# ChuWeiEr/GravInv3DHMC

Measured on AMD Instinct MI355X. Metric: HMC leapfrog steps/sec + G·ρ achieved HBM GB/s at 1/2/4/8 GPUs, higher is better.
Workload: dtype f64

## Files before the change

gravinv3dhmc_amd/_lib.py:

```python
import ctypes as C
import os

import numpy as np

_HERE = os.path.dirname(os.path.abspath(__file__))
LIB_PATH = os.environ.get("GRAVHMC_LIB") or os.path.join(_HERE, "libgravhmc.so")

GH_OK, GH_ERR_ARG, GH_ERR_HIP, GH_ERR_NOMEM, GH_ERR_OVERFLOW, GH_ERR_UNSUPPORTED, GH_ERR_COMM = \
    0, -1, -2, -3, -4, -5, -6
CELL_PRISM, CELL_TESSEROID, CELL_PRISM_TF, CELL_PRISM_COMP, CELL_TESSEROID_COMP, CELL_PRISM_JOINT = 0, 1, 2, 3, 4, 5
CELL_PRISM_MULTI = 6
CELL_PRISM_MVI = 7
CELL_PRISM_MVI_DATA = 8
CELL_TESS_MVI_DATA = 9
CELL_TESSEROID_MULTI = 10
BCOMP_TF, BCOMP_BX, BCOMP_BY, BCOMP_BZ = range(4)
BCOMPONENTS = {"tf": BCOMP_TF, "bx": BCOMP_BX, "by": BCOMP_BY, "bz": BCOMP_BZ}
BCOMP_MAX = 4
MULTI_MAX = 11
COMP_POTENTIAL, COMP_GEOID, COMP_GX, COMP_GY, COMP_GZ, COMP_GXX, COMP_GXY, COMP_GXZ, COMP_GYY, COMP_GYZ, COMP_GZZ = \
    range(11)
COMPONENTS = {"potential": COMP_POTENTIAL, "geoid": COMP_GEOID, "gx": COMP_GX, "gy": COMP_GY, "gz": COMP_GZ,
              "gxx": COMP_GXX, "gxy": COMP_GXY, "gxz": COMP_GXZ, "gyy": COMP_GYY, "gyz": COMP_GYZ, "gzz": COMP_GZZ}
REG_KINDS = {"Damping": 0, "Smoothness": 1, "MS": 2, "TV": 3}
# ... 111 lines not shown
    "gh_shard_unique_id": (C.c_int, [C.c_void_p]),
    "gh_shard_init": (C.c_int, [_ctx, C.c_void_p, C.c_int, C.c_int, _i64, _i64]),
    "gh_shard_init_callback": (C.c_int, [_ctx, C.c_void_p, C.c_void_p, C.c_int, C.c_int, _i64, _i64]),
    "gh_shard_init_rows": (C.c_int, [_ctx, C.c_void_p, C.c_int, C.c_int, _i64, _i64]),
    "gh_shard_init_rows_callback": (C.c_int, [_ctx, C.c_void_p, C.c_void_p, C.c_int, C.c_int, _i64, _i64]),
    "gh_shard_allreduce": (C.c_int, [_ctx, _dp, _i64]),
    "gh_rng_create": (C.c_int, [C.POINTER(C.c_void_p), C.c_uint32]),
    "gh_rng_destroy": (None, [C.c_void_p]),
    "gh_rng_set_threads": (C.c_int, [C.c_void_p, C.c_int]),
    "gh_host_cores": (C.c_int, []),
    "gh_rng_set_state": (C.c_int, [C.c_void_p, C.POINTER(C.c_uint32), C.c_int, C.c_int, C.c_double]),
    "gh_rng_get_state": (C.c_int, [C.c_void_p, C.POINTER(C.c_uint32), C.POINTER(C.c_int), C.POINTER(C.c_int),
                                   C.POINTER(C.c_double)]),
    "gh_rng_draw_trajectories": (C.c_int, [C.c_void_p, C.c_int, C.c_int, C.c_int, _i64, C.c_double,
                                           C.POINTER(C.c_int), _dp, _dp]),
    "gh_format_row_fixed8": (C.c_int64, [_dp, _i64, C.c_char_p, _i64]),
    "gh_measure_stream_read": (C.c_int, [_ctx, C.c_int, C.c_int, C.POINTER(C.c_double)]),
    "gh_profile_enable": (C.c_int, [_ctx, C.c_int]),
    "gh_fold_info": (C.c_int, [_ctx, C.POINTER(C.c_int), C.POINTER(C.c_int), C.POINTER(_i64), C.POINTER(C.c_double),
                               C.POINTER(C.c_double)]),
    "gh_fold_detect": (C.c_int, [_i64, _dp, _dp, _dp, _i64, _dp, C.POINTER(C.c_int), C.POINTER(C.c_int)]),
    "gh_fold_pair_info": (C.c_int, [_ctx, C.POINTER(C.c_int), C.POINTER(C.c_int), C.POINTER(_i64), C.POINTER(_i64),
                                    C.POINTER(_i64)]),
    "gh_fold_detect_pair": (C.c_int, [_i64, _dp, _dp, _dp, _i64, _dp, C.POINTER(C.c_int), C.POINTER(C.c_int),
                                      C.POINTER(C.c_int), C.POINTER(_i64), C.POINTER(C.c_int)]),
    "gh_fold_pair_rows": (C.c_int, [_i64, _dp, _dp, _dp, _i64, _dp, C.POINTER(C.c_int), C.POINTER(C.c_int),
                                    C.POINTER(C.c_int), C.POINTER(C.c_int), C.POINTER(_i64), C.POINTER(C.c_int)]),
    "gh_profile_read": (C.c_int, [_ctx, C.POINTER(C.c_double), C.POINTER(_i64),
                                  C.POINTER(_i64)]),
    "gh_set_translation_invariant": (C.c_int, [_ctx, C.c_int]),
# ... 62 lines not shown
```

gravinv3dhmc_amd/csrc/gravhmc.hip:

```cpp
#include "../../include/gravhmc.h"
#include "kernels.hip.h"
#include "batch.hip.h"
#include "bscg.hip.h"
#include "exchange.hip.h"
#include "resident.hip.h"
#include "resbatch.hip.h"
#include "teamsweep.hip.h"
#include "mfbatch.hip.h"
#include "batchteam.hip.h"
#include "lonsym.hip.h"
#include "lonsymh.hip.h"
#include "lonres.hip.h"
#include "lonsymw.hip.h"
#include "fold.hip.h"
#include "lattice.hip.h"
#include "latbatch.hip.h"
#include "poststream.hip.h"
#include "tessmag.hip.h"

#include <dlfcn.h>
#include <rccl/rccl.h>

#include <algorithm>
#include <array>
#include <atomic>
#include <cfloat>
#include <chrono>
#include <climits>
#include <cmath>
#include <cstdarg>
#include <cstdio>
#include <cstdlib>
#include <cstring>
#include <functional>
#include <map>
#include <mutex>
#include <string>
#include <utility>
#include <thread>
#include <vector>

using namespace ghk;
static_assert(COMP_POTENTIAL == GH_COMP_POTENTIAL && COMP_GEOID == GH_COMP_GEOID && COMP_GX == GH_COMP_GX &&
                  COMP_GY == GH_COMP_GY && COMP_GZ == GH_COMP_GZ && COMP_GXX == GH_COMP_GXX && COMP_GXY == GH_COMP_GXY &&
                  COMP_GXZ == GH_COMP_GXZ && COMP_GYY == GH_COMP_GYY && COMP_GYZ == GH_COMP_GYZ &&
                  COMP_GZZ == GH_COMP_GZZ,
              "the kernels' component numbers are the C ABI's GH_COMP_*");
static_assert(MULTI_MAX == GH_MULTI_MAX, "the kernels' row-block table holds the C ABI's GH_MULTI_MAX components");
static_assert(BCOMP_MAX == GH_BCOMP_MAX && BCOMP_MAX <= MULTI_MAX && BCOMP_TF == GH_BCOMP_TF && BCOMP_BX == GH_BCOMP_BX &&
                  BCOMP_BY == GH_BCOMP_BY && BCOMP_BZ == GH_BCOMP_BZ,
              "the kernels' data components are the C ABI's GH_BCOMP_*");

#include "host_rows.h"
#include "host_ctx.h"
#include "host_cells.h"
#include "host_sweep.h"
#include "host_fold.h"
#include "host_lattice.h"
#include "host_lonsym.h"
#include "host_comm.h"
#include "host_wavelet.h"
#include "host_eval.h"
#include "host_poststream.h"
#include "host_resident.h"
#include "host_resbatch.h"
#include "host_lonres.h"
#include "host_batch.h"
#include "host_batchrun.h"
// ... 49 lines not shown
    if (c->stream) hipStreamSynchronize(c->stream);
    if (c->sh.comm) {
        std::string err;
        RcclApi *api = rccl_api(err);
        if (api && api->CommDestroy) api->CommDestroy(c->sh.comm);
    }
    if (c->sh.hbuf) hipHostFree(c->sh.hbuf);
    if (c->bt.h) hipHostFree(c->bt.h);
    traj_lists_free(c->rs.lists);
    traj_lists_free(c->rs.ls.lists);
    if (c->ls) {
        traj_lists_free(c->ls->res.lists);
        if (c->ls->res.ev0) hipEventDestroy(c->ls->res.ev0);
        if (c->ls->res.ev1) hipEventDestroy(c->ls->res.ev1);
    }
    for (PinnedBlock &pm : c->pinned) hipHostFree(pm.base);
    for (void *p : c->allocs) hipFree(p);
    if (c->h_scal) hipHostFree(c->h_scal);
    for (hipEvent_t ev : c->ev) hipEventDestroy(ev);
    if (c->copy_ev) hipEventDestroy(c->copy_ev);
    if (c->copy_stream) hipStreamDestroy(c->copy_stream);
    if (c->rs.ev0) hipEventDestroy(c->rs.ev0);
    if (c->rs.ev1) hipEventDestroy(c->rs.ev1);
    if (c->stream) hipStreamDestroy(c->stream);
    delete c->ls;
    delete c->lat;
    delete c;
}

int gh_device_info(const gh_ctx *c, char *name256, int *cus, int64_t *mem_bytes)
// ... 1426 lines not shown
    HIPCHK(c, hipMemsetAsync(c->wv.coeff, 0, sizeof(double) * (size_t)c->wv.Mp, c->stream));
    TRY(run_dwt(c, c->tmpM, c->M, 1, c->wv.coeff, c->wv.s1, c->wv.s2));
    return d2h(c, coeff, c->wv.coeff, (size_t)c->wv.Mp);
}

int gh_forward_wavelet(gh_ctx *c, const double *mw, double *dpre)
{
    if (!c || !mw || !dpre) return fail(c, GH_ERR_ARG, "gh_forward_wavelet: null pointer");
    TRY(need(c, c->wv.on, "gh_forward_wavelet: call gh_compress_wavelet first"));
    HIPCHK(c, hipSetDevice(c->device));
    TRY(h2d(c, c->tmpM, mw, (size_t)c->M));
    TRY(wavelet_forward(c, c->tmpM, c->tmpN));
    return d2h(c, dpre, c->tmpN, (size_t)c->N);
}

int gh_chain_init(gh_ctx *c, const double *x0, const double *low, const double *high)
{
    if (!c || !x0 || !low || !high) return fail(c, GH_ERR_ARG, "gh_chain_init: null pointer");
    TRY(need(c, c->have_G && c->have_data && c->have_reg,
             "gh_chain_init: needs a kernel matrix, gh_set_data and gh_set_reg"));
    HIPCHK(c, hipSetDevice(c->device));
    TRY(ensure_work(c));
    c->cur = 0;
    c->xcur = 0;
    c->spec_valid = c->pn_valid = false;
    c->st_stale = false;
    c->accept_count = 0;
    TRY(h2d(c, c->xb[0], x0, (size_t)c->M));
    TRY(h2d(c, c->low, low, (size_t)c->M));
    TRY(h2d(c, c->high, high, (size_t)c->M));
    TRY(eval_forward(c, c->xb[0], c->st[0]));
    TRY(scal_ready(c, c->st[0]));
    TRY(d2h(c, c->h_scal, c->st[0].scal, 4));
    c->cg.phi_cur = 0.0;
    if (coupling_on(c)) {
        TRY(d2h(c, c->h_scal + 8, c->st[0].phi, 1));
        c->cg.phi_cur = c->h_scal[8];
    }
    c->cg.phi_last = c->cg.phi_cur;
    TRY(lonsym_epilogue_check(c));
    c->U_cur[0] = c->h_scal[2];
    c->U_cur[1] = c->h_scal[0];
    c->U_cur[2] = c->h_scal[1];
    c->chain_ready = true;
    return GH_OK;
}

int gh_chain_prefetch_momentum(gh_ctx *c, const double *p0_next)
{
    if (!c || !p0_next) return fail(c, GH_ERR_ARG, "gh_chain_prefetch_momentum: null pointer");
    TRY(need(c, c->chain_ready, "gh_chain_prefetch_momentum: call gh_chain_init first"));
    HIPCHK(c, hipSetDevice(c->device));
    TRY(h2d(c, c->pn, p0_next, (size_t)c->M));
    sumsq_kernel<<<dim3(c->n_pp0), dim3(256), 0, c->stream>>>(c->pn, c->M, c->pp0_part);
    {
        std::vector<double> part((size_t)c->n_pp0);
        TRY(d2h(c, part.data(), c->pp0_part, (size_t)c->n_pp0));
        double s = 0.0;
        for (double v : part) s += v;
// ... 489 lines not shown
    const gh_ctx::Resident::LockStep &b = c->rs.ls;
    if (launches) *launches = b.launches;
    if (lock_steps) *lock_steps = b.lock_steps;
    if (chain_steps) *chain_steps = b.chain_steps;
    if (lost_steps) *lost_steps = b.lost;
    if (timeouts) *timeouts = b.xg.aborts;
    return GH_OK;
}

int gh_pinned_alloc(gh_ctx *c, size_t bytes, void **host)
{
    if (!c || !host || bytes == 0) return fail(c, GH_ERR_ARG, "gh_pinned_alloc: null pointer or no bytes");
    HIPCHK(c, hipSetDevice(c->device));
    void *p = nullptr;
    HIPCHK(c, hipHostMalloc(&p, bytes));
    c->pinned.push_back({(char *)p, bytes});
    *host = p;
    return GH_OK;
}

int gh_pinned_free(gh_ctx *c, void *host)
{
    if (!c || !host) return fail(c, GH_ERR_ARG, "gh_pinned_free: null pointer");
    for (size_t i = 0; i < c->pinned.size(); ++i)
        if (c->pinned[i].base == (char *)host) {
            HIPCHK(c, hipSetDevice(c->device));
            if (c->stream) HIPCHK(c, hipStreamSynchronize(c->stream));
            HIPCHK(c, hipHostFree(host));
            c->pinned.erase(c->pinned.begin() + (long)i);
            return GH_OK;
// ... 301 lines not shown
    std::vector<std::thread> th;
    for (int t = 1; t < T; ++t) th.emplace_back(work, t);
    work(0);
    for (std::thread &x : th) x.join();
    int64_t pos = 0;
    for (int t = 0; t < T; ++t) {
        if (len[(size_t)t] < 0 || pos + len[(size_t)t] > cap) return -1;
        memcpy(out + pos, buf[(size_t)t].data(), (size_t)len[(size_t)t]);
        pos += len[(size_t)t];
    }
    return pos;
}

#include "host_rng.h"

int gh_profile_enable(gh_ctx *c, int enable)
{
    if (!c) return GH_ERR_ARG;
    HIPCHK(c, hipSetDevice(c->device));
    if (enable && c->ev.empty()) {
        c->ev.resize(8192);
        for (auto &e : c->ev) HIPCHK(c, hipEventCreate(&e));
        c->ev_bytes.assign(c->ev.size() / 2, 0);
    }
    for (gh_ctx *k : c->kids) TRY(gh_profile_enable(k, enable));
    c->prof = enable != 0;
    c->prof_stride = (c->ld * c->M * 8 < (int64_t)(1 << 30)) ? 16 : 1;
    c->prof_seen = 0;
    c->ev_used = 0;
    c->prof_ms_acc = 0.0;
// ... 147 lines not shown
```

gravinv3dhmc_amd/csrc/host_chain.h:

```cpp
#pragma once

static int chain_state_fresh(gh_ctx *c)
{
    if (!c->st_stale) return GH_OK;
    TRY(eval_forward(c, c->xb[c->xcur], c->st[c->cur]));
    TRY(scal_ready(c, c->st[c->cur]));
    TRY(d2h(c, c->h_scal, c->st[c->cur].scal, 4));
    c->U_cur[0] = c->h_scal[2];
    c->U_cur[1] = c->h_scal[0];
    c->U_cur[2] = c->h_scal[1];
    c->st_stale = false;
    return GH_OK;
}

static inline int other_of3(int a, int b)
{
    for (int i = 0; i < 3; ++i)
        if (i != a && i != b) return i;
    return 0;
}

static int chain_trajectory_impl(gh_ctx *c, const double *p0, double dt, int L, double u, const double *p0_next,
                                 int *accepted, double out5[5])
{
    if (!c || !p0 || !accepted || !out5) return fail(c, GH_ERR_ARG, "gh_chain_trajectory: null pointer");
    TRY(need(c, c->chain_ready, "gh_chain_trajectory: call gh_chain_init first"));
    if (L < 1) return fail(c, GH_ERR_ARG, "gh_chain_trajectory: L must be >= 1");
    HIPCHK(c, hipSetDevice(c->device));
    TRY(chain_state_fresh(c));
    struct TeamsOk {
        gh_ctx *c;
        ~TeamsOk() { c->chain_teams_ok = false; }
    } teams_guard{c};
    c->chain_teams_ok = true;
    const size_t M = (size_t)c->M;
    const int nt = c->n_teams;
    const bool use_spec = c->spec_valid && c->spec_dt == dt && p0[0] == c->spec_probe[0] &&
// ... 29 lines not shown
        a.low = c->low;
        a.high = c->high;
        a.c_u = (s == 0) ? dt * 0.5 : dt;
        a.dt = dt;
        a.slab = c->slab;
        TRY(launch_sweep(c, a));
        TRY(finalize(c, c->xb[xout], c->st[sout]));
        xin = xout;
        pin ^= 1;
        sin = sout;
    }
    bool spec = c->pn_valid;
    double probe[3] = {c->pn_probe[0], c->pn_probe[1], c->pn_probe[2]};
    double pn_pp0 = c->pn_pp0;
    bool pn_deferred = false;
    if (p0_next) {
        if (!c->copy_stream) {
            HIPCHK(c, hipStreamCreateWithFlags(&c->copy_stream, hipStreamNonBlocking));
            HIPCHK(c, hipEventCreateWithFlags(&c->copy_ev, hipEventDisableTiming));
        }
        HIPCHK(c, hipMemcpyAsync(c->pn, p0_next, M * sizeof(double), hipMemcpyHostToDevice, c->copy_stream));
        HIPCHK(c, hipEventRecord(c->copy_ev, c->copy_stream));
        HIPCHK(c, hipStreamWaitEvent(c->stream, c->copy_ev, 0));
        sumsq_kernel<<<dim3(c->n_pp0), dim3(256), 0, c->stream>>>(c->pn, c->M, c->pn0_part);
        probe[0] = p0_next[0];
        probe[1] = p0_next[c->M / 2];
        probe[2] = p0_next[c->M - 1];
        spec = true;
        pn_deferred = true;
    }
// ... 34 lines not shown
                                 c->stream));
    }
    if (!use_spec)
        HIPCHK(c, hipMemcpyAsync(h + 16 + 2 * nt, c->pp0_part, (size_t)c->n_pp0 * sizeof(double),
                                 hipMemcpyDeviceToHost, c->stream));
    if (pn_deferred)
        HIPCHK(c, hipMemcpyAsync(h + 16 + 2 * nt + c->n_pp0, c->pn0_part, (size_t)c->n_pp0 * sizeof(double),
                                 hipMemcpyDeviceToHost, c->stream));
    HIPCHK(c, hipStreamSynchronize(c->stream));
    TRY(lonsym_epilogue_check(c));
    bool failed = false;
    TRY(team_failed(c, &failed));
    if (!failed) TRY(mft_failed(c, &failed));
    auto redo = [&]() -> int {
        c->spec_valid = c->pn_valid = false;
        const int rc = chain_trajectory_impl(c, p0, dt, L, u, p0_next, accepted, out5);
        team_resume(c);
        return rc;
    };
    if (failed && c->sh.kind == 0) return redo();
    if (pn_deferred) {
        double s = 0.0;
        for (int t = 0; t < c->n_pp0; ++t) s += h[16 + 2 * nt + c->n_pp0 + t];
        pn_pp0 = s;
    }
    double pp1 = 0.0, pp0 = 0.0;
    for (int t = 0; t < nt; ++t) pp1 += h[16 + t];
    if (use_spec)
        pp0 = c->spec_pp0;
    else
        for (int t = 0; t < c->n_pp0; ++t) pp0 += h[16 + 2 * nt + t];
// ... 22 lines not shown
            c->spec_x = xs;
            c->spec_p = pin ^ 1;
            c->spec_set = ss;
            c->spec_probe[0] = probe[0];
            c->spec_probe[1] = probe[1];
            c->spec_probe[2] = probe[2];
        }
    } else if (spec) {
        c->spec_misses += 1;
    }
    c->pn_valid = false;
    *accepted = acc ? 1 : 0;
    c->cg.phi_last = c->cg.phi_cur;
    return GH_OK;
}
```

gravinv3dhmc_amd/csrc/host_ctx.h:

```cpp
#pragma once

static thread_local std::string g_create_error;

struct LonSymHost;
struct LatticeHost;

struct DevBuf {
    void *p = nullptr;
    size_t bytes = 0;
};

struct ExchangeGuard {
    unsigned *abort_w = nullptr;
    unsigned seen[4] = {0, 0, 0, 0};
    unsigned tag = 0, tagE = 0, ltag = 0;
    std::vector<DevBuf> grans;
    bool dirty = false;
    bool inflight = false;
    int aborts = 0;
};

struct TrajLists {
    int cap = 0;
    int *L = nullptr, *accepted = nullptr, *chain = nullptr;
// ... 309 lines not shown
        size_t lds = 0;
        double max_dev = 0.0, build_ms = 0.0;
        int64_t launches = 0;
        bool exact = false;
        bool pair_detected = false, pair_on = false;
        int pair_reason = GH_FOLD_PAIR_UNDECIDED;
        int64_t n_work = 0, n_pairs = 0, work_per_team = 0;
        int pair_rows = 0;
        bool pair_rows_ok = false;
        int *wtab_d = nullptr, *row_tau_d = nullptr, *orb_tau_d = nullptr;
        int *ptab_d = nullptr, *row_code_d = nullptr;
    } fd;

    std::vector<PinnedBlock> pinned;

    double *ring = nullptr, *ring_mean = nullptr, *ring_sd = nullptr;
    int ring_K = 0, ring_next = 0;
    int64_t ring_count = 0;

    struct PostStream {
        bool on = false;
        int slot = 0;
        int64_t from = 0, count = 0;
        ghk::PostState d = {};
        double *lo = nullptr, *hi = nullptr, *iw = nullptr;
        double *row = nullptr;
        double *out = nullptr;
        double *qout = nullptr;
        size_t qout_n = 0;
        int64_t n[16] = {}, K[16] = {};
// ... 192 lines not shown
```

gravinv3dhmc_amd/csrc/host_rng.h:

```cpp
#pragma once

static const int RNG_BLOCKS = 8;

#if defined(__x86_64__) && !defined(__HIP_DEVICE_COMPILE__)
#define GH_HOST_CLONES __attribute__((target_clones("avx512f", "avx2", "default")))
#else
#define GH_HOST_CLONES
#endif

struct gh_rng {
    uint32_t keys[RNG_BLOCKS][624];
    uint32_t out[RNG_BLOCKS * 624];
    int nb;
    int p;
    int has_gauss;
    double gauss;
    std::vector<double> r2;
    int threads = 0;
};

GH_HOST_CLONES static void rng_twist(const uint32_t *in, uint32_t *mt)
{
    if (mt != in) memcpy(mt, in, 624 * sizeof(uint32_t));
    int i;
// ... 253 lines not shown
```

gravinv3dhmc_amd/engine.py:

```python
import collections
import ctypes as C

import numpy as np

from . import _lib
from ._lib import check, f64, ptr


Store = collections.namedtuple("Store", "kind cols rows table")


class DeviceMatrix(object):

    def __init__(self, engine):
        self._engine = engine
        self.shape = (engine.N, engine.M)
        self.dtype = np.dtype(np.float64)
        self.ndim = 2

    def to_numpy(self):
        eng = self._engine
        if eng.joint:
            H = eng.download_G()
            n, m = eng.N // 2, eng.M // 2
# ... 589 lines not shown
        import threading
        if batch is None:
            batch = self.default_batch()
        pool = self.__dict__.setdefault("_p0_pool", {"i": 0, "blocks": []})

        def p0_block(n, width):
            if n * width * 8 * 3 > (2 << 30) or n < 2:
                return np.empty((n, width))
            if not pool["blocks"] or pool["blocks"][0].shape[1] != width or pool["blocks"][0].shape[0] < n:
                for b in pool["blocks"]:
                    self.pinned_free(b)
                pool["blocks"] = [self.pinned_empty((max(n, batch), width)) for _ in range(3)]
            pool["i"] = (pool["i"] + 1) % 3
            return pool["blocks"][pool["i"]][:n]

        if hasattr(draws, "take_block"):
            def take(n, head=None):
                if head is None:
                    if n < 2:
                        return draws.take_block(n)
                    out = (np.empty(n, dtype=np.int32), p0_block(n, draws.M), np.empty(n))
                    got = len(draws.take_block(n, out=out, at=0)[0])
                    return tuple(o[:got] for o in out)
                out = (np.empty(n, dtype=np.int32), p0_block(n, head[1].shape[1]), np.empty(n))
                out[0][0], out[1][0], out[2][0] = head[0][0], head[1][0], head[2][0]
                got = len(draws.take_block(n - 1, out=out, at=1)[0]) if n > 1 else 0
                return tuple(o[:1 + got] for o in out)
        else:
            it = iter(draws)

            def take(n, head=None):
# ... 14 lines not shown
                blk = p0_block(len(ps), ps[0].shape[0])
                for i, pv in enumerate(ps):
                    blk[i] = pv
                return (np.asarray(Ls, dtype=np.int32), blk, np.asarray(us, dtype=np.float64))

        import queue
        jobs = queue.Queue()

        def worker():
            while True:
                item = jobs.get()
                if item is None:
                    return
                prepared, res, entered, done = item
                try:
                    res["n"] = self._run_batch(prepared, dt, stop_at_accepts, record_from, want_x, entered)
                except BaseException as e:
                    res["e"] = e
                finally:
                    entered.set()
                    done.set()

        th = threading.Thread(target=worker, daemon=True)
        th.start()

        def start(prepared):
            res = {"a": prepared}
            entered, done = threading.Event(), threading.Event()
            jobs.put((prepared, res, entered, done))
            entered.wait()
            return done, res

        def finish(job):
            job[0].wait()
            if "e" in job[1]:
                raise job[1]["e"]
            return job[1]["n"], job[1]["a"]

        def some(blk):
            return blk is not None and len(blk[0]) > 0

        try:
            cur = take(1 if self.M * 8 >= (1 << 20) else batch)
            look = take(1) if some(cur) else None
            look = look if some(look) else None
            job = start(self._prepare_batch(cur, look, want_x)) if some(cur) else None
            while some(cur):
                nxt = take(batch, head=look) if look is not None else None
                nlook = take(1) if some(nxt) else None
                nlook = nlook if some(nlook) else None
                nprepared = self._prepare_batch(nxt, nlook, want_x) if some(nxt) else None
                n_run, a = finish(job)
                short = n_run < len(cur[0])
                job = start(nprepared) if (overlap and some(nxt) and not short) else None
                stop = False
                acc, out5, xs = a["acc"], a["out5"], a["xs"]
                for k in range(n_run):
                    x = xs[k].copy() if (want_x and acc[k]) else None
                    if on_result(int(cur[0][k]), bool(acc[k]), out5[k],
                                 self._full_vec(x) if x is not None else None) is False:
                        stop = True
                        break
                if stop or short or not some(nxt):
                    if job is not None:
                        finish(job)
                    break
                if job is None:
                    job = start(nprepared)
                cur, look = nxt, nlook
        finally:
            jobs.put(None)
            th.join()

    def chain_get_x(self):
        x = np.empty(self.M)
        self._chk(self._lib.gh_chain_get_x(self._h, ptr(x)))
        return x

    def chain_get_dsyn(self):
        d = np.empty(self.N)
        self._chk(self._lib.gh_chain_get_dsyn(self._h, ptr(d)))
        return d

    def batch_init(self, x0s, low, high):
        x0s = np.ascontiguousarray(np.atleast_2d(x0s), dtype=np.float64)
        if x0s.ndim != 2 or x0s.shape[1] != self.M:
            raise ValueError("x0s must be (C, M)")
# ... 221 lines not shown
```

gravinv3dhmc_amd/inversion/rng.py:

```python
import ctypes as C

import numpy as np

from .. import _lib


def draw_workers(n_chains):
    return int(max(1, min(int(n_chains), _lib.load().gh_host_cores() - 3)))


class LegacyDraws(object):

    def __init__(self, M, Lrange, Sigma, fixed_L=None, limit=None, seed=None, helpers=None):
        self._lib = _lib.load()
        self.M = int(M)
        self.Lmin, self.Lmax = int(Lrange[0]), int(Lrange[1])
        sig = np.asarray(Sigma, dtype=np.float64)
        self._sigma = float(sig) if sig.ndim == 0 else 1.0
        self._sigma_vec = None if sig.ndim == 0 else np.ascontiguousarray(np.broadcast_to(sig, (self.M,)))
        self._plan = None if fixed_L is None else list(fixed_L)
        self._left = limit if self._plan is None else len(self._plan)
        self._h = C.c_void_p()
        self._own = seed is not None
        if self._lib.gh_rng_create(C.byref(self._h), int(seed) if self._own else 0) != 0:
# ... 60 lines not shown
                                                    us.ctypes.data_as(dp))
        else:
            rc = self._lib.gh_rng_draw_trajectories(self._h, n, 0, 0, self.M, self._sigma,
                                                    Ls.ctypes.data_as(ip), p0s.ctypes.data_as(dp),
                                                    us.ctypes.data_as(dp))
            done = len(self._plan) - self._left
            Ls[:] = self._plan[done:done + n]
        if rc != 0:
            raise RuntimeError("gh_rng_draw_trajectories failed (%d)" % rc)
        if self._sigma_vec is not None:
            p0s *= self._sigma_vec
        if self._left is not None:
            self._left -= n
        return Ls, p0s, us

    def use_ring(self, engine, rows):
        self._ring_engine = engine
        self._ring = engine.pinned_empty((int(rows), self.M))
        self._ring_Ls = np.empty(int(rows), dtype=np.int32)
        self._ring_us = np.empty(int(rows))
        self._ring_head = 0
        self._ring_base = self._ring.ctypes.data
        return self

    def take_ring(self, n):
        rows = self._ring.shape[0]
        if n > rows:
            raise ValueError("take_ring: more rows than the ring holds")
        out, stride = [], self.M * 8
        while n > 0:
# ... 24 lines not shown
```

include/gravhmc.h:

```cpp
#ifndef GRAVHMC_H
#define GRAVHMC_H

#include <stdint.h>

#ifdef __cplusplus
extern "C" {
#endif

typedef struct gh_ctx gh_ctx;

typedef enum {
    GH_OK = 0,
    GH_ERR_ARG = -1,
    GH_ERR_HIP = -2,
    GH_ERR_NOMEM = -3,
    GH_ERR_OVERFLOW = -4,
    GH_ERR_UNSUPPORTED = -5,
    GH_ERR_COMM = -6
} gh_status;

enum { GH_CELL_PRISM = 0, GH_CELL_TESSEROID = 1, GH_CELL_PRISM_TF = 2, GH_CELL_PRISM_COMP = 3, GH_CELL_TESSEROID_COMP = 4,
       GH_CELL_PRISM_JOINT = 5, GH_CELL_PRISM_MULTI = 6, GH_CELL_PRISM_MVI = 7, GH_CELL_PRISM_MVI_DATA = 8 };
enum { GH_CELL_TESS_MVI_DATA = 9, GH_CELL_TESSEROID_MULTI = 10 };
enum { GH_BCOMP_TF = 0, GH_BCOMP_BX = 1, GH_BCOMP_BY = 2, GH_BCOMP_BZ = 3 };
// ... 157 lines not shown

int64_t gh_format_row_fixed8(const double *v, int64_t n, char *out, int64_t cap);


typedef struct gh_rng gh_rng;
int gh_rng_create(gh_rng **out, uint32_t seed);
void gh_rng_destroy(gh_rng *rng);
int gh_rng_set_state(gh_rng *rng, const uint32_t *key624, int pos, int has_gauss, double cached);
int gh_rng_get_state(const gh_rng *rng, uint32_t *key624, int *pos, int *has_gauss, double *cached);
int gh_rng_set_threads(gh_rng *rng, int threads);
int gh_host_cores(void);
int gh_rng_draw_trajectories(gh_rng *rng, int K, int Lmin, int Lmax, int64_t M, double sigma, int *L,
                             double *p0s , double *us );


enum {
    GH_FOLD_ON = 0,
    GH_FOLD_UNDECIDED = 1,
    GH_FOLD_SWITCHED_OFF = 2,
    GH_FOLD_NOT_GZ = 3,
    GH_FOLD_OBS = 4,
    GH_FOLD_CELLS = 5,
    GH_FOLD_FIXED = 6,
    GH_FOLD_SMALL = 7,
    GH_FOLD_PATH = 8,
    GH_FOLD_NOMEM = 9,
    GH_FOLD_DEVIATION = 10
};
int gh_fold_info(const gh_ctx *ctx, int *on, int *reason, int64_t *store_bytes, double *max_dev, double *build_ms);
int gh_fold_detect(int64_t N, const double *x, const double *y, const double *z, int64_t M, const double *bounds6,
// ... 49 lines not shown
```

Baseline: 1024.

## Feed chain momenta from a producer thread into a pinned ring

```diff
diff --git a/gravinv3dhmc_amd/_lib.py b/gravinv3dhmc_amd/_lib.py
--- a/gravinv3dhmc_amd/_lib.py
+++ b/gravinv3dhmc_amd/_lib.py
@@ -149,6 +149,15 @@
                                    C.POINTER(C.c_double)]),
     "gh_rng_draw_trajectories": (C.c_int, [C.c_void_p, C.c_int, C.c_int, C.c_int, _i64, C.c_double,
                                            C.POINTER(C.c_int), _dp, _dp]),
+    "gh_chain_feed_force": (C.c_int, [_ctx, C.c_int]),
+    "gh_chain_feed_ring": (C.c_int, [_ctx, C.POINTER(C.c_int)]),
+    "gh_chain_feed_open": (C.c_int, [_ctx, C.c_void_p, C.c_int, C.c_int, C.POINTER(C.c_int), _i64, C.c_double, _dp,
+                                     C.POINTER(C.c_void_p)]),
+    "gh_chain_feed_grant": (C.c_int, [C.c_void_p, _i64]),
+    "gh_chain_feed_close": (C.c_int, [C.c_void_p]),
+    "gh_chain_feed_stats": (C.c_int, [_ctx, C.POINTER(_i64), C.POINTER(C.c_double)]),
+    "gh_chain_run_fed": (C.c_int, [_ctx, C.c_void_p, C.c_int, C.c_double, _i64, _i64, C.POINTER(C.c_int), _dp,
+                                   C.POINTER(C.c_int), _dp, C.POINTER(C.c_int)]),
     "gh_format_row_fixed8": (C.c_int64, [_dp, _i64, C.c_char_p, _i64]),
     "gh_measure_stream_read": (C.c_int, [_ctx, C.c_int, C.c_int, C.POINTER(C.c_double)]),
     "gh_profile_enable": (C.c_int, [_ctx, C.c_int]),
diff --git a/gravinv3dhmc_amd/csrc/gravhmc.hip b/gravinv3dhmc_amd/csrc/gravhmc.hip
--- a/gravinv3dhmc_amd/csrc/gravhmc.hip
+++ b/gravinv3dhmc_amd/csrc/gravhmc.hip
@@ -27,6 +27,7 @@
 #include <cfloat>
 #include <chrono>
 #include <climits>
+#include <condition_variable>
 #include <cmath>
 #include <cstdarg>
 #include <cstdio>
@@ -52,6 +53,7 @@
               "the kernels' data components are the C ABI's GH_BCOMP_*");
 
 #include "host_rows.h"
+#include "host_feed.h"
 #include "host_ctx.h"
 #include "host_cells.h"
 #include "host_sweep.h"
@@ -131,6 +133,11 @@
         if (c->ls->res.ev0) hipEventDestroy(c->ls->res.ev0);
         if (c->ls->res.ev1) hipEventDestroy(c->ls->res.ev1);
     }
+    if (c->feed) {
+        feed_close(c->feed);
+        c->feed = nullptr;
+    }
+    feed_ring_release(c->feed_ring);
     for (PinnedBlock &pm : c->pinned) hipHostFree(pm.base);
     for (void *p : c->allocs) hipFree(p);
     if (c->h_scal) hipHostFree(c->h_scal);
@@ -1587,6 +1594,54 @@
     return d2h(c, dpre, c->tmpN, (size_t)c->N);
 }
 
+static void *feed_alloc_pinned(size_t bytes)
+{
+    void *p = nullptr;
+    if (hipHostMalloc(&p, bytes) != hipSuccess) {
+        (void)hipGetLastError();
+        return nullptr;
+    }
+    return p;
+}
+
+static void feed_free_pinned(void *p) { (void)hipHostFree(p); }
+
+static bool chain_on_sweep_path(gh_ctx *c)
+{
+    return c->sh.kind == 0 && !c->wv.on && c->kids.empty() && !lonres_usable(c) && !resident_usable(c);
+}
+
+static int chain_feed_batch(int64_t M) { return (int)std::max<int64_t>(4, std::min<int64_t>(128, ((int64_t)6 << 20) / (8 * M))); }
+
+static void chain_feed_ring(gh_ctx *c)
+{
+    if (c->feed) return;
+    const bool want = env_int("GRAVHMC_CHAIN_FEED", 1) != 0 && (c->feed_force || c->M * 8 >= ((int64_t)1 << 20)) &&
+                      chain_on_sweep_path(c);
+    if (!want) return;
+    const int64_t cap = ((int64_t)256 << 20) / (c->M * 8);
+    const int R = (int)std::min<int64_t>(c->feed_force >= 2 ? c->feed_force : 2 * chain_feed_batch(c->M) + 2, cap);
+    if (R < 2) return;
+    const int64_t before = c->feed_ring.allocs;
+    if (!feed_ring_reserve(c->feed_ring, R, c->M, feed_alloc_pinned, feed_free_pinned)) return;
+    c->host_allocs += c->feed_ring.allocs - before;
+    if (!c->copy_stream) {
+        if (hipStreamCreateWithFlags(&c->copy_stream, hipStreamNonBlocking) != hipSuccess ||
+            hipEventCreateWithFlags(&c->copy_ev, hipEventDisableTiming) != hipSuccess) {
+            (void)hipGetLastError();
+            if (c->copy_stream) (void)hipStreamDestroy(c->copy_stream);
+            c->copy_stream = nullptr;
+            c->copy_ev = nullptr;
+            return;
+        }
+    }
+    if (c->feed_ring.allocs != before && c->pn) {
+        if (hipMemcpyAsync(c->pn, c->feed_ring.rows, (size_t)c->M * sizeof(double), hipMemcpyHostToDevice, c->copy_stream) != hipSuccess ||
+            hipStreamSynchronize(c->copy_stream) != hipSuccess)
+            (void)hipGetLastError();
+    }
+}
+
 int gh_chain_init(gh_ctx *c, const double *x0, const double *low, const double *high)
 {
     if (!c || !x0 || !low || !high) return fail(c, GH_ERR_ARG, "gh_chain_init: null pointer");
@@ -1616,6 +1671,9 @@
     c->U_cur[1] = c->h_scal[0];
     c->U_cur[2] = c->h_scal[1];
     c->chain_ready = true;
+    chain_feed_ring(c);
+    c->host_allocs_init = c->host_allocs;
+    c->feed_done = gh_ctx::FeedCounters();
     return GH_OK;
 }
 
@@ -2135,6 +2193,7 @@
     HIPCHK(c, hipSetDevice(c->device));
     void *p = nullptr;
     HIPCHK(c, hipHostMalloc(&p, bytes));
+    c->host_allocs += 1;
     c->pinned.push_back({(char *)p, bytes});
     *host = p;
     return GH_OK;
@@ -2466,6 +2525,152 @@
 
 #include "host_rng.h"
 
+
+int gh_chain_feed_force(gh_ctx *c, int rows)
+{
+    if (!c || rows < 0) return GH_ERR_ARG;
+    c->feed_force = rows;
+    return GH_OK;
+}
+
+int gh_chain_feed_ring(gh_ctx *c, int *rows)
+{
+    if (!c || !rows) return GH_ERR_ARG;
+    *rows = 0;
+    if (c->chain_ready && c->feed_ring.rows && c->feed_ring.M == c->M && !c->feed && chain_on_sweep_path(c))
+        *rows = c->feed_ring.R;
+    return GH_OK;
+}
+
+int gh_chain_feed_open(gh_ctx *c, gh_rng *rng, int Lmin, int Lmax, const int *plan, int64_t n_plan, double sigma,
+                       const double *sigma_vec, gh_chain_feed **feed)
+{
+    if (!c || !rng || !feed) return fail(c, GH_ERR_ARG, "gh_chain_feed_open: null pointer");
+    *feed = nullptr;
+    TRY(need(c, c->chain_ready, "gh_chain_feed_open: call gh_chain_init first"));
+    if (c->feed) return fail(c, GH_ERR_ARG, "gh_chain_feed_open: the context's feed is open already");
+    if (!c->feed_ring.rows || c->feed_ring.M != c->M)
+        return fail(c, GH_ERR_ARG, "gh_chain_feed_open: the context has no momentum ring (gh_chain_feed_ring)");
+    gh_chain_feed *f = feed_open(&c->feed_ring, rng, Lmin, Lmax, plan, n_plan, sigma, sigma_vec);
+    if (!f) return fail(c, GH_ERR_ARG, "gh_chain_feed_open: bad arguments or no memory");
+    f->owner = c;
+    c->feed = f;
+    *feed = f;
+    return GH_OK;
+}
+
+int gh_chain_feed_grant(gh_chain_feed *f, int64_t n)
+{
+    if (!f || n < 0) return GH_ERR_ARG;
+    feed_grant(f, n);
+    return GH_OK;
+}
+
+int gh_chain_feed_close(gh_chain_feed *f)
+{
+    if (!f) return GH_OK;
+    gh_ctx *c = static_cast<gh_ctx *>(f->owner);
+    if (c) {
+        if (c->stream) {
+            hipSetDevice(c->device);
+            hipStreamSynchronize(c->stream);
+            if (c->copy_stream) hipStreamSynchronize(c->copy_stream);
+        }
+        c->feed = nullptr;
+    }
+    const int64_t waits_own = f->waits_own, waits_look = f->waits_look;
+    const double own_s = f->wait_own_s, look_s = f->wait_look_s;
+    const int64_t granted = f->granted;
+    const bool threaded = f->threaded;
+    const int rc = feed_close(f);
+    if (c) {
+        c->feed_done.rows += granted;
+        c->feed_done.waits_own += waits_own;
+        c->feed_done.waits_look += waits_look;
+        c->feed_done.wait_own_s += own_s;
+        c->feed_done.wait_look_s += look_s;
+        c->feed_done.threaded = threaded;
+        if (rc != GH_OK) return fail(c, rc, "gh_chain_feed_close: a draw failed (%d)", rc);
+    }
+    return rc;
+}
+
+int gh_chain_feed_stats(gh_ctx *c, int64_t out[8], double secs[2])
+{
+    if (!c || !out || !secs) return GH_ERR_ARG;
+    gh_ctx::FeedCounters s = c->feed_done;
+    int64_t threaded = s.threaded ? 1 : 0;
+    if (gh_chain_feed *f = c->feed) {
+        std::lock_guard<std::mutex> lk(f->mu);
+        s.rows += f->drawn;
+        s.waits_own += f->waits_own;
+        s.waits_look += f->waits_look;
+        s.wait_own_s += f->wait_own_s;
+        s.wait_look_s += f->wait_look_s;
+        threaded = f->threaded ? 1 : 0;
+    }
+    out[0] = s.rows;
+    out[1] = s.waits_own;
+    out[2] = s.waits_look;
+    out[3] = c->host_allocs - c->host_allocs_init;
+    out[4] = threaded;
+    out[5] = c->feed_ring.rows ? c->feed_ring.R : 0;
+    out[6] = c->feed ? 1 : 0;
+    out[7] = 0;
+    secs[0] = s.wait_own_s;
+    secs[1] = s.wait_look_s;
+    return GH_OK;
+}
+
+struct FedLook {
+    gh_chain_feed *f;
+    int64_t idx;
+};
+
+static const double *fed_lookahead(void *arg)
+{
+    FedLook *q = static_cast<FedLook *>(arg);
+    const double *row = nullptr;
+    (void)feed_row(q->f, q->idx, true, &row, nullptr, nullptr);
+    return row;
+}
+
+int gh_chain_run_fed(gh_ctx *c, gh_chain_feed *f, int K, double dt, int64_t stop_at_accepts, int64_t record_from,
+                     int *accepted, double *out5s, int *Ls_out, double *x_out, int *n_run)
+{
+    if (!c || !f || K < 1 || !accepted || !out5s || !n_run) return fail(c, GH_ERR_ARG, "gh_chain_run_fed: bad arguments");
+    TRY(need(c, c->chain_ready, "gh_chain_run_fed: call gh_chain_init first"));
+    TRY(need(c, c->feed == f, "gh_chain_run_fed: not this context's open feed"));
+    TRY(need(c, chain_on_sweep_path(c), "gh_chain_run_fed: this chain does not run on the sweep path (use gh_chain_run)"));
+    const size_t M = (size_t)c->M;
+    *n_run = 0;
+    if (stop_at_accepts > 0 && c->accept_count >= stop_at_accepts) return GH_OK;
+    for (int k = 0; k < K; ++k) {
+        const int64_t idx = f->next;
+        const double *p0 = nullptr;
+        int L = 0;
+        double u = 0.0;
+        const int rc = feed_row(f, idx, false, &p0, &L, &u);
+        if (rc != GH_OK) return fail(c, rc, "gh_chain_run_fed: drawing a trajectory failed (%d)", rc);
+        if (!p0) break;
+        FedLook look{f, idx + 1};
+        P0Next nx;
+        nx.late = fed_lookahead;
+        nx.arg = &look;
+        TRY(chain_trajectory_late(c, p0, dt, L, u, nx, &accepted[k], out5s + 5 * k));
+        if (Ls_out) Ls_out[k] = L;
+        f->next = idx + 1;
+        feed_release(f, idx + 1);
+        *n_run = k + 1;
+        if (accepted[k]) {
+            TRY(chain_accept_row(c, c, c->xb[c->xcur], record_from, x_out ? x_out + (size_t)k * M : nullptr));
+            if (stop_at_accepts > 0 && c->accept_count >= stop_at_accepts) break;
+        }
+    }
+    HIPCHK(c, hipStreamSynchronize(c->stream));
+    return GH_OK;
+}
+
 int gh_profile_enable(gh_ctx *c, int enable)
 {
     if (!c) return GH_ERR_ARG;
diff --git a/gravinv3dhmc_amd/csrc/host_chain.h b/gravinv3dhmc_amd/csrc/host_chain.h
--- a/gravinv3dhmc_amd/csrc/host_chain.h
+++ b/gravinv3dhmc_amd/csrc/host_chain.h
@@ -20,7 +20,13 @@
     return 0;
 }
 
-static int chain_trajectory_impl(gh_ctx *c, const double *p0, double dt, int L, double u, const double *p0_next,
+struct P0Next {
+    const double *ptr = nullptr;
+    const double *(*late)(void *arg) = nullptr;
+    void *arg = nullptr;
+};
+
+static int chain_trajectory_late(gh_ctx *c, const double *p0, double dt, int L, double u, const P0Next &nx,
                                  int *accepted, double out5[5])
 {
     if (!c || !p0 || !accepted || !out5) return fail(c, GH_ERR_ARG, "gh_chain_trajectory: null pointer");
@@ -80,6 +86,7 @@
     double probe[3] = {c->pn_probe[0], c->pn_probe[1], c->pn_probe[2]};
     double pn_pp0 = c->pn_pp0;
     bool pn_deferred = false;
+    const double *p0_next = nx.late ? nx.late(nx.arg) : nx.ptr;
     if (p0_next) {
         if (!c->copy_stream) {
             HIPCHK(c, hipStreamCreateWithFlags(&c->copy_stream, hipStreamNonBlocking));
@@ -144,7 +151,7 @@
     if (!failed) TRY(mft_failed(c, &failed));
     auto redo = [&]() -> int {
         c->spec_valid = c->pn_valid = false;
-        const int rc = chain_trajectory_impl(c, p0, dt, L, u, p0_next, accepted, out5);
+        const int rc = chain_trajectory_late(c, p0, dt, L, u, nx, accepted, out5);
         team_resume(c);
         return rc;
     };
@@ -197,3 +204,11 @@
     c->cg.phi_last = c->cg.phi_cur;
     return GH_OK;
 }
+
+static int chain_trajectory_impl(gh_ctx *c, const double *p0, double dt, int L, double u, const double *p0_next,
+                                 int *accepted, double out5[5])
+{
+    P0Next nx;
+    nx.ptr = p0_next;
+    return chain_trajectory_late(c, p0, dt, L, u, nx, accepted, out5);
+}
diff --git a/gravinv3dhmc_amd/csrc/host_ctx.h b/gravinv3dhmc_amd/csrc/host_ctx.h
--- a/gravinv3dhmc_amd/csrc/host_ctx.h
+++ b/gravinv3dhmc_amd/csrc/host_ctx.h
@@ -347,6 +347,17 @@
 
     std::vector<PinnedBlock> pinned;
 
+    FeedRing feed_ring;
+    int feed_force = 0;
+    gh_chain_feed *feed = nullptr;
+    int64_t host_allocs = 0;
+    int64_t host_allocs_init = 0;
+    struct FeedCounters {
+        int64_t rows = 0, waits_own = 0, waits_look = 0;
+        double wait_own_s = 0.0, wait_look_s = 0.0;
+        bool threaded = false;
+    } feed_done;
+
     double *ring = nullptr, *ring_mean = nullptr, *ring_sd = nullptr;
     int ring_K = 0, ring_next = 0;
     int64_t ring_count = 0;
diff --git a/gravinv3dhmc_amd/csrc/host_feed.h b/gravinv3dhmc_amd/csrc/host_feed.h
--- /dev/null
+++ b/gravinv3dhmc_amd/csrc/host_feed.h
@@ -0,0 +1,233 @@
+#pragma once
+
+typedef void *(*feed_alloc_fn)(size_t bytes);
+typedef void (*feed_free_fn)(void *p);
+
+struct FeedRing {
+    double *rows = nullptr;
+    int R = 0;
+    int64_t M = 0;
+    feed_free_fn free_fn = nullptr;
+    int64_t allocs = 0;
+};
+
+static void feed_ring_release(FeedRing &g)
+{
+    if (g.rows && g.free_fn) g.free_fn(g.rows);
+    g.rows = nullptr;
+    g.R = 0;
+    g.M = 0;
+}
+
+static bool feed_ring_reserve(FeedRing &g, int R, int64_t M, feed_alloc_fn alloc_fn, feed_free_fn free_fn)
+{
+    if (g.rows && g.M == M && g.R == R) return true;
+    feed_ring_release(g);
+    if (R < 2 || M < 1 || !alloc_fn) return false;
+    void *p = alloc_fn((size_t)R * (size_t)M * sizeof(double));
+    if (!p) return false;
+    g.rows = static_cast<double *>(p);
+    g.R = R;
+    g.M = M;
+    g.free_fn = free_fn;
+    g.allocs += 1;
+    return true;
+}
+
+struct gh_chain_feed {
+    FeedRing *ring = nullptr;
+    gh_rng *rng = nullptr;
+    int Lmin = 0, Lmax = 0;
+    bool has_plan = false;
+    std::vector<int> plan;
+    double sigma = 1.0;
+    std::vector<double> sigma_vec;
+    std::vector<int> Ls;
+    std::vector<double> us;
+    std::mutex mu;
+    std::condition_variable cv_prod, cv_cons;
+    int64_t granted = 0, drawn = 0, freed = 0;
+    int64_t next = 0;
+    bool closing = false;
+    bool threaded = false;
+    int rc = GH_OK;
+    std::thread th;
+    void *owner = nullptr;
+    int64_t waits_own = 0, waits_look = 0;
+    double wait_own_s = 0.0, wait_look_s = 0.0;
+};
+
+static int feed_draw_one(gh_chain_feed *f, int64_t idx)
+{
+#pragma clang fp contract(off)
+    const int64_t M = f->ring->M;
+    const size_t slot = (size_t)(idx % f->ring->R);
+    double *row = f->ring->rows + slot * (size_t)M;
+    int L = 0;
+    double u = 0.0;
+    int rc;
+    try {
+        if (f->has_plan) {
+            rc = gh_rng_draw_trajectories(f->rng, 1, 0, 0, M, f->sigma, &L, row, &u);
+            L = (size_t)idx < f->plan.size() ? f->plan[(size_t)idx] : 0;
+        } else {
+            rc = gh_rng_draw_trajectories(f->rng, 1, f->Lmin, f->Lmax, M, f->sigma, &L, row, &u);
+        }
+    } catch (...) {
+        rc = GH_ERR_NOMEM;
+    }
+    if (rc != GH_OK) return rc;
+    if (!f->sigma_vec.empty()) {
+        const double *sv = f->sigma_vec.data();
+        for (int64_t i = 0; i < M; ++i) row[i] = row[i] * sv[i];
+    }
+    f->Ls[slot] = L;
+    f->us[slot] = u;
+    return GH_OK;
+}
+
+static void feed_producer(gh_chain_feed *f)
+{
+    std::unique_lock<std::mutex> lk(f->mu);
+    for (;;) {
+        f->cv_prod.wait(lk, [&] {
+            return f->rc != GH_OK || (f->drawn < f->granted && f->drawn - f->freed < f->ring->R) ||
+                   (f->closing && f->drawn >= f->granted);
+        });
+        if (f->rc != GH_OK || f->drawn >= f->granted) return;
+        const int64_t idx = f->drawn;
+        lk.unlock();
+        const int rc = feed_draw_one(f, idx);
+        lk.lock();
+        if (rc != GH_OK) {
+            f->rc = rc;
+            f->cv_cons.notify_all();
+            return;
+        }
+        f->drawn = idx + 1;
+        if (f->closing) f->freed = f->drawn;
+        f->cv_cons.notify_all();
+    }
+}
+
+static bool feed_spawn_thread(gh_chain_feed *f)
+{
+    try {
+        f->th = std::thread(feed_producer, f);
+        return true;
+    } catch (...) {
+        return false;
+    }
+}
+static bool (*feed_spawn)(gh_chain_feed *) = feed_spawn_thread;
+
+static gh_chain_feed *feed_open(FeedRing *ring, gh_rng *rng, int Lmin, int Lmax, const int *plan, int64_t n_plan,
+                                double sigma, const double *sigma_vec)
+{
+    if (!ring || !ring->rows || ring->R < 2 || !rng || (!plan && Lmax < Lmin) || (plan && n_plan < 0)) return nullptr;
+    gh_chain_feed *f = nullptr;
+    try {
+        f = new gh_chain_feed();
+        f->ring = ring;
+        f->rng = rng;
+        f->Lmin = Lmin;
+        f->Lmax = Lmax;
+        f->has_plan = plan != nullptr;
+        if (plan) f->plan.assign(plan, plan + n_plan);
+        f->sigma = sigma;
+        if (sigma_vec) f->sigma_vec.assign(sigma_vec, sigma_vec + ring->M);
+        f->Ls.assign((size_t)ring->R, 0);
+        f->us.assign((size_t)ring->R, 0.0);
+    } catch (...) {
+        delete f;
+        return nullptr;
+    }
+    f->threaded = feed_spawn(f);
+    return f;
+}
+
+static int64_t feed_grant(gh_chain_feed *f, int64_t n)
+{
+    std::lock_guard<std::mutex> lk(f->mu);
+    if (n > 0) f->granted += n;
+    if (f->has_plan && f->granted > (int64_t)f->plan.size()) f->granted = (int64_t)f->plan.size();
+    f->cv_prod.notify_one();
+    return f->granted;
+}
+
+static int feed_row(gh_chain_feed *f, int64_t idx, bool lookahead, const double **row, int *L, double *u)
+{
+    *row = nullptr;
+    std::unique_lock<std::mutex> lk(f->mu);
+    if (idx >= f->granted || idx < f->freed) return f->rc;
+    if (f->drawn <= idx && f->rc == GH_OK) {
+        const auto t0 = std::chrono::steady_clock::now();
+        if (f->threaded) {
+            f->cv_cons.wait(lk, [&] { return f->drawn > idx || f->rc != GH_OK; });
+        } else {
+            while (f->drawn <= idx && f->rc == GH_OK) {
+                if (f->drawn - f->freed >= f->ring->R) {
+                    f->rc = GH_ERR_ARG;
+                    break;
+                }
+                const int64_t at = f->drawn;
+                lk.unlock();
+                const int rc = feed_draw_one(f, at);
+                lk.lock();
+                if (rc != GH_OK)
+                    f->rc = rc;
+                else
+                    f->drawn = at + 1;
+            }
+        }
+        const double dt = std::chrono::duration<double>(std::chrono::steady_clock::now() - t0).count();
+        if (lookahead) {
+            f->waits_look += 1;
+            f->wait_look_s += dt;
+        } else {
+            f->waits_own += 1;
+            f->wait_own_s += dt;
+        }
+    }
+    if (f->rc != GH_OK) return f->rc;
+    const size_t slot = (size_t)(idx % f->ring->R);
+    *row = f->ring->rows + slot * (size_t)f->ring->M;
+    if (L) *L = f->Ls[slot];
+    if (u) *u = f->us[slot];
+    return GH_OK;
+}
+
+static void feed_release(gh_chain_feed *f, int64_t upto)
+{
+    std::lock_guard<std::mutex> lk(f->mu);
+    if (upto > f->drawn) upto = f->drawn;
+    if (upto > f->freed) f->freed = upto;
+    f->cv_prod.notify_one();
+}
+
+static int feed_close(gh_chain_feed *f)
+{
+    if (!f) return GH_OK;
+    {
+        std::unique_lock<std::mutex> lk(f->mu);
+        f->closing = true;
+        f->freed = f->drawn;
+        if (!f->threaded) {
+            while (f->drawn < f->granted && f->rc == GH_OK) {
+                const int64_t at = f->drawn;
+                lk.unlock();
+                const int rc = feed_draw_one(f, at);
+                lk.lock();
+                if (rc != GH_OK)
+                    f->rc = rc;
+                else
+                    f->freed = f->drawn = at + 1;
+            }
+        }
+        f->cv_prod.notify_one();
+    }
+    if (f->th.joinable()) f->th.join();
+    const int rc = f->rc;
+    delete f;
+    return rc;
+}
diff --git a/gravinv3dhmc_amd/csrc/host_rng.h b/gravinv3dhmc_amd/csrc/host_rng.h
--- a/gravinv3dhmc_amd/csrc/host_rng.h
+++ b/gravinv3dhmc_amd/csrc/host_rng.h
@@ -2,7 +2,8 @@
 
 static const int RNG_BLOCKS = 8;
 
-#if defined(__x86_64__) && !defined(__HIP_DEVICE_COMPILE__)
+#if defined(GH_HOST_CLONES)
+#elif defined(__x86_64__) && !defined(__HIP_DEVICE_COMPILE__)
 #define GH_HOST_CLONES __attribute__((target_clones("avx512f", "avx2", "default")))
 #else
 #define GH_HOST_CLONES
diff --git a/gravinv3dhmc_amd/engine.py b/gravinv3dhmc_amd/engine.py
--- a/gravinv3dhmc_amd/engine.py
+++ b/gravinv3dhmc_amd/engine.py
@@ -1,5 +1,6 @@
 import collections
 import ctypes as C
+import os
 
 import numpy as np
 
@@ -627,7 +628,30 @@
             pool["i"] = (pool["i"] + 1) % 3
             return pool["blocks"][pool["i"]][:n]
 
-        if hasattr(draws, "take_block"):
+        prepare, run_batch = self._prepare_batch, self._run_batch
+        feed = self._feed_open(draws)
+        if feed is not None:
+            lib = self._lib
+
+            def take(n, head=None):
+                got = draws.feed_granted(n - (0 if head is None else 1))
+                if got > 0:
+                    self._chk(lib.gh_chain_feed_grant(feed, got))
+                return (np.zeros(got + (0 if head is None else 1), dtype=np.int32), None, None)
+
+            def prepare(blk, look, want_x):
+                K = len(blk[0])
+                return {"K": K, "Ls": blk[0], "acc": (C.c_int * K)(), "out5": np.empty((K, 5)),
+                        "xs": np.empty((K, self.M)) if want_x else None, "n_run": C.c_int(0)}
+
+            def run_batch(a, dt, stop_at, record_from, want_x, entered=None):
+                if entered is not None:
+                    entered.set()
+                self._chk(lib.gh_chain_run_fed(self._h, feed, a["K"], float(dt), int(stop_at), int(record_from),
+                                               a["acc"], ptr(a["out5"]), a["Ls"].ctypes.data_as(C.POINTER(C.c_int)),
+                                               ptr(a["xs"]), C.byref(a["n_run"])))
+                return a["n_run"].value
+        elif hasattr(draws, "take_block"):
             def take(n, head=None):
                 if head is None:
                     if n < 2:
@@ -672,7 +696,7 @@
                     return
                 prepared, res, entered, done = item
                 try:
-                    res["n"] = self._run_batch(prepared, dt, stop_at_accepts, record_from, want_x, entered)
+                    res["n"] = run_batch(prepared, dt, stop_at_accepts, record_from, want_x, entered)
                 except BaseException as e:
                     res["e"] = e
                 finally:
@@ -702,12 +726,12 @@
             cur = take(1 if self.M * 8 >= (1 << 20) else batch)
             look = take(1) if some(cur) else None
             look = look if some(look) else None
-            job = start(self._prepare_batch(cur, look, want_x)) if some(cur) else None
+            job = start(prepare(cur, look, want_x)) if some(cur) else None
             while some(cur):
                 nxt = take(batch, head=look) if look is not None else None
                 nlook = take(1) if some(nxt) else None
                 nlook = nlook if some(nlook) else None
-                nprepared = self._prepare_batch(nxt, nlook, want_x) if some(nxt) else None
+                nprepared = prepare(nxt, nlook, want_x) if some(nxt) else None
                 n_run, a = finish(job)
                 short = n_run < len(cur[0])
                 job = start(nprepared) if (overlap and some(nxt) and not short) else None
@@ -729,6 +753,37 @@
         finally:
             jobs.put(None)
             th.join()
+            if feed is not None:
+                self._lib.gh_chain_feed_close(feed)
+
+    def chain_feed_force(self, rows=1):
+        self._chk(self._lib.gh_chain_feed_force(self._h, int(rows)))
+
+    def chain_feed_rows(self):
+        rows = C.c_int(0)
+        self._chk(self._lib.gh_chain_feed_ring(self._h, C.byref(rows)))
+        return rows.value
+
+    def chain_feed_stats(self):
+        out, secs = (C.c_int64 * 8)(), (C.c_double * 2)()
+        self._chk(self._lib.gh_chain_feed_stats(self._h, out, secs))
+        return {"rows_drawn": out[0], "waits_own_row": out[1], "waits_lookahead": out[2], "wait_own_row_s": secs[0],
+                "wait_lookahead_s": secs[1], "allocations": out[3], "producer_thread": bool(out[4]),
+                "ring_rows": out[5], "open": bool(out[6])}
+
+    def _feed_open(self, draws):
+        if not hasattr(draws, "feed_source") or os.environ.get("GRAVHMC_CHAIN_FEED", "1") == "0":
+            return None
+        if getattr(draws, "M", None) != self.M or self.chain_feed_rows() < 1:
+            return None
+        src = draws.feed_source()
+        plan = None if src["plan"] is None else np.ascontiguousarray(src["plan"], dtype=np.int32)
+        feed = C.c_void_p()
+        self._chk(self._lib.gh_chain_feed_open(
+            self._h, src["handle"], int(src["Lmin"]), int(src["Lmax"]),
+            plan.ctypes.data_as(C.POINTER(C.c_int)) if plan is not None else None, len(plan) if plan is not None else 0,
+            float(src["sigma"]), ptr(src["sigma_vec"]), C.byref(feed)))
+        return feed
 
     def chain_get_x(self):
         x = np.empty(self.M)
diff --git a/gravinv3dhmc_amd/inversion/rng.py b/gravinv3dhmc_amd/inversion/rng.py
--- a/gravinv3dhmc_amd/inversion/rng.py
+++ b/gravinv3dhmc_amd/inversion/rng.py
@@ -98,6 +98,19 @@
             self._left -= n
         return Ls, p0s, us
 
+    def feed_source(self):
+        plan = None if self._plan is None else self._plan[len(self._plan) - self._left:]
+        return {"handle": self._h, "Lmin": self.Lmin, "Lmax": self.Lmax, "plan": plan, "sigma": self._sigma,
+                "sigma_vec": self._sigma_vec}
+
+    def feed_granted(self, n):
+        if self._left is not None:
+            n = min(n, self._left)
+        n = max(int(n), 0)
+        if self._left is not None:
+            self._left -= n
+        return n
+
     def use_ring(self, engine, rows):
         self._ring_engine = engine
         self._ring = engine.pinned_empty((int(rows), self.M))
diff --git a/include/gravhmc.h b/include/gravhmc.h
--- a/include/gravhmc.h
+++ b/include/gravhmc.h
@@ -195,6 +195,18 @@
                              double *p0s , double *us );
 
 
+typedef struct gh_chain_feed gh_chain_feed;
+int gh_chain_feed_force(gh_ctx *ctx, int rows);
+int gh_chain_feed_ring(gh_ctx *ctx, int *rows);
+int gh_chain_feed_open(gh_ctx *ctx, gh_rng *rng, int Lmin, int Lmax, const int *plan, int64_t n_plan, double sigma,
+                       const double *sigma_vec, gh_chain_feed **feed);
+int gh_chain_feed_grant(gh_chain_feed *feed, int64_t n);
+int gh_chain_feed_close(gh_chain_feed *feed);
+int gh_chain_feed_stats(gh_ctx *ctx, int64_t out[8], double secs[2]);
+int gh_chain_run_fed(gh_ctx *ctx, gh_chain_feed *feed, int K, double dt, int64_t stop_at_accepts,
+                     int64_t record_from, int *accepted, double *out5s, int *Ls_out, double *x_out, int *n_run);
+
+
 enum {
     GH_FOLD_ON = 0,
     GH_FOLD_UNDECIDED = 1,
diff --git a/profiles/chain_feed_stats.py b/profiles/chain_feed_stats.py
--- /dev/null
+++ b/profiles/chain_feed_stats.py
@@ -0,0 +1,25 @@
+#!/usr/bin/env python3
+import json
+import os
+import sys
+
+ROOT = os.path.dirname(os.path.dirname(os.path.abspath(__file__)))
+sys.path.insert(0, ROOT)
+
+import bench
+from gravinv3dhmc_amd.engine import Engine
+
+_run_chain = Engine.run_chain
+
+
+def run_chain(self, *a, **kw):
+    try:
+        return _run_chain(self, *a, **kw)
+    finally:
+        print("chain_feed_stats " + json.dumps(self.chain_feed_stats()), flush=True)
+
+
+Engine.run_chain = run_chain
+
+if __name__ == "__main__":
+    bench.main()
diff --git a/profiles/chain_timeline.py b/profiles/chain_timeline.py
--- /dev/null
+++ b/profiles/chain_timeline.py
@@ -0,0 +1,62 @@
+#!/usr/bin/env python3
+import argparse
+import csv
+import glob
+import json
+import os
+
+
+def load(d):
+    rows = []
+    for f in sorted(glob.glob(os.path.join(d, "**", "*kernel_trace.csv"), recursive=True)):
+        for r in csv.DictReader(open(f)):
+            rows.append((int(r["Start_Timestamp"]), int(r["End_Timestamp"]), r["Kernel_Name"]))
+    rows.sort()
+    return rows
+
+
+def gaps(rows, is_sweep, floor_ns):
+    out, seen = [], 0
+    for (s0, e0, n0), (s1, e1, n1) in zip(rows, rows[1:]):
+        seen += 1 if is_sweep(n0) else 0
+        if s1 - e0 > floor_ns:
+            out.append({"after_sweeps": seen, "ms": round((s1 - e0) / 1e6, 3), "after": n0[:48], "before": n1[:48]})
+    return out
+
+
+def main():
+    ap = argparse.ArgumentParser()
+    ap.add_argument("dir")
+    ap.add_argument("out")
+    ap.add_argument("--sweeps", type=int, default=61)
+    ap.add_argument("--gap-ms", type=float, default=0.2)
+    ap.add_argument("--sweep-name", default="fold_pair_sweep")
+    ap.add_argument("--stop-name", default="stream_read")
+    a = ap.parse_args()
+    rows = load(a.dir)
+
+    def is_sweep(name):
+        return a.sweep_name in name
+
+    at = [i for i, r in enumerate(rows) if is_sweep(r[2])]
+    if len(at) < a.sweeps:
+        raise SystemExit("only %d sweeps in the trace" % len(at))
+    first = at[-a.sweeps]
+    stop = next((i for i in range(at[-1], len(rows)) if a.stop_name in rows[i][2]), len(rows))
+    reg = rows[first:stop]
+    span = reg[-1][1] - reg[0][0]
+    busy = sum(e - s for s, e, _ in reg)
+    sweeps_ms = [(e - s) / 1e6 for s, e, n in reg if is_sweep(n)]
+    res = {"sweeps_in_region": a.sweeps, "kernels_in_region": len(reg),
+           "span_ms": round(span / 1e6, 3), "kernel_ms": round(busy / 1e6, 3), "idle_ms": round((span - busy) / 1e6, 3),
+           "sweep_ms": {"mean": round(sum(sweeps_ms) / len(sweeps_ms), 4), "min": round(min(sweeps_ms), 4),
+                        "max": round(max(sweeps_ms), 4)},
+           "sweep_ms_each": [round(v, 3) for v in sweeps_ms],
+           "gaps_in_region": gaps(reg, is_sweep, a.gap_ms * 1e6),
+           "gaps_whole_run_from_first_sweep": gaps(rows[at[0]:], is_sweep, a.gap_ms * 1e6)}
+    json.dump(res, open(a.out, "w"), indent=1)
+    print(json.dumps({k: v for k, v in res.items() if k not in ("sweep_ms_each", "gaps_whole_run_from_first_sweep")}))
+
+
+if __name__ == "__main__":
+    main()
```

After: 1063 (median of 6 runs). 1.04x the previous value.
